# zhuker/lamejs

Measured on NVIDIA H100. Metric: encoded audio seconds/sec (44.1kHz stereo 128kbps CBR), higher is better.
Workload: dtype f64

## Files before the change

lamejs_b200/csrc/k_quant.cuh:

```cuda
#ifndef MP3B200_K_QUANT_CUH
#define MP3B200_K_QUANT_CUH
#include <stddef.h>
#include "mp3_device.cuh"
#include "mp3_tables.h"
#include "k_psy.cuh"

#define Q_LARGE_BITS 100000
#define Q_IXMAX 8206
#define Q_FULL 0xffffffffu

struct GranuleInfoDev {
  int global_gain, part2_3_length, part2_length, big_values, count1, scalefac_compress;
  int table_select[3], region0_count, region1_count, preflag, scalefac_scale, count1table_select, block_type;
  int subblock_gain[4];
  int count1bits, sfbmax, sfbdivide, sfb_lmax, psymax, psy_lmax, sfb_smin, max_nonzero_coeff;
  int scalefac[MP3_SFBMAX];
  int slen[4];
  int part_row;
  int pad_;
  double xrpow_max;
};
struct QuantFrameState {
  int stream, rel_frame;
  int in_old[2], in_step[2];
  int out_old[2], out_step[2];
  int bs_gain0[2], bs_step0[2];
  int used0[2];
  unsigned long long bs_hash[2][2];
  int scfsi[2][4];
  int redo;
  int valid;
};
#define Q_R0(ch) (1 << (ch))
#define Q_R1S(ch) (4 << (ch))
#define Q_R1(ch) (16 << (ch))
#define Q_R0_ANY 3
#define Q_R1_ANY 48
#define Q_R1S_ANY 12
struct GcPrep { float xmin[MP3_SFBMAX]; int have, mnz, block_type; double xrpow_max; };

__device__ unsigned short g_huff_code[1666];
__device__ unsigned char g_huff_len[1666];
__constant__ int c_huff_off[34];
__constant__ int c_huff_xlen[34];
__device__ int g_t32l[16];
__device__ int g_t33l[16];
__constant__ int c_slen1_n[16];
__constant__ int c_slen2_n[16];
__device__ int g_slen_n[2][16];
__device__ int g_scale_tab[2][16];
__device__ unsigned int g_cat_tab[8][256];
__constant__ int c_slen1_tab[16];
__constant__ int c_slen2_tab[16];
__constant__ int c_huf_noesc[15];

static int quant_upload_constants() {
  static const int t32l[16] = {1, 5, 5, 7, 5, 8, 7, 9, 5, 7, 7, 9, 7, 9, 9, 10};
  static const int t33l[16] = {4, 5, 5, 6, 5, 6, 6, 7, 5, 6, 6, 7, 6, 7, 7, 8};
  static const int s1n[16] = {1, 1, 1, 1, 8, 2, 2, 2, 4, 4, 4, 8, 8, 8, 16, 16};
  static const int s2n[16] = {1, 2, 4, 8, 1, 2, 4, 8, 2, 4, 8, 2, 4, 8, 4, 8};
  static const int s1t[16] = {0, 0, 0, 0, 3, 1, 1, 1, 2, 2, 2, 3, 3, 3, 4, 4};
  static const int s2t[16] = {0, 1, 2, 3, 0, 1, 2, 3, 1, 2, 3, 1, 2, 3, 2, 3};
  static const int ss[16] = {0, 18, 36, 54, 54, 36, 54, 72, 54, 72, 90, 72, 90, 108, 108, 126};
  static const int sl[16] = {0, 10, 20, 30, 33, 21, 31, 41, 32, 42, 52, 43, 53, 63, 64, 74};
  static const int hn[15] = {1, 2, 5, 7, 7, 10, 10, 13, 13, 13, 13, 13, 13, 13, 13};
#define UP(sym, src) if (cudaMemcpyToSymbol(sym, src, sizeof(src)) != cudaSuccess) return -100
  UP(g_huff_code, MP3_HUFF_CODE); UP(g_huff_len, MP3_HUFF_LEN); UP(c_huff_off, MP3_HUFF_OFF);
  UP(c_huff_xlen, MP3_HUFF_XLEN);
  UP(g_t32l, t32l); UP(g_t33l, t33l); UP(c_slen1_n, s1n); UP(c_slen2_n, s2n);
  UP(c_slen1_tab, s1t); UP(c_slen2_tab, s2t); UP(c_huf_noesc, hn);
  {
    static int sn[2][16], st[2][16];
    static unsigned int ct[8][256];
    for (int k = 0; k < 16; k++) { sn[0][k] = s1n[k]; sn[1][k] = s2n[k]; st[0][k] = sl[k]; st[1][k] = ss[k]; }
    static const int fam[6] = {1, 2, 5, 7, 10, 13};
    for (int x = 0; x < 16; x++) for (int y = 0; y < 16; y++) {
      const int q = x * 16 + y;
      for (int c = 0; c < 6; c++) {
        const int t1 = fam[c], xl = MP3_HUFF_XLEN[t1];
        unsigned a = 0, b = 0, d = 0;
        if (x < xl && y < xl) {
          const int i = x * xl + y;
          if (c == 0) a = b = d = MP3_HUFF_LEN[MP3_HUFF_OFF[1] + i];
          else if (c == 1) { a = MP3_HUFF_TABLE23[i] >> 16; b = d = MP3_HUFF_TABLE23[i] & 0xffff; }
          else if (c == 2) { a = MP3_HUFF_TABLE56[i] >> 16; b = d = MP3_HUFF_TABLE56[i] & 0xffff; }
          else { a = MP3_HUFF_LEN[MP3_HUFF_OFF[t1] + i]; b = MP3_HUFF_LEN[MP3_HUFF_OFF[t1 + 1] + i]; d = MP3_HUFF_LEN[MP3_HUFF_OFF[t1 + 2] + i]; }
        }
        ct[c][q] = a | (b << 11) | (d << 22);
      }
      { const unsigned a = MP3_HUFF_LARGETBL[q] >> 16, b = MP3_HUFF_LARGETBL[q] & 0xffff; ct[6][q] = a | (b << 11) | (b << 22); }
      ct[7][q] = 0;
    }
    UP(g_slen_n, sn); UP(g_scale_tab, st); UP(g_cat_tab, ct);
  }
#undef UP
  return 0;
}

struct __align__(16) GcWork {
  float xrpow[576];
  short ixw[576];
  short* ixg;
  GranuleInfoDev w, b;
  const Mp3Geo* geo;
  float xmin[MP3_SFBMAX], distort[MP3_SFBMAX];
  int pn_step[MP3_SFBMAX]; float pn_noise[MP3_SFBMAX], pn_noise_log[MP3_SFBMAX];
  int pn_global_gain, pn_sfb_count1;
  unsigned char mode[MP3_SFBMAX + 1];
  short nstart[MP3_SFBMAX], nlen[MP3_SFBMAX];
  int scratch[8];
  double dscratch[4];
  __align__(16) float xr[576];
};
struct __align__(16) WarpShared {
  double ath[6];
  int scfsi[4];
  GcWork wk;
};
#define Q_STRIDE_NOXR ((int)((offsetof(WarpShared, wk) + offsetof(GcWork, xr) + 15) & ~(size_t)15))
static_assert((offsetof(WarpShared, wk) + offsetof(GcWork, xr)) % 16 == 0 && (offsetof(WarpShared, wk) + offsetof(GcWork, xrpow)) % 16 == 0 &&
              (offsetof(WarpShared, wk) + offsetof(GcWork, ixw)) % 16 == 0 && sizeof(WarpShared) % 16 == 0, "rows are moved as 16-byte vectors");
#ifndef Q_SLIM_BLOCKS
#define Q_SLIM_BLOCKS 9
#endif

#define LANE (threadIdx.x & 31)
#ifdef Q_TASKSTAT
__device__ int g_taskstat[1 << 16][8];
#endif
#ifdef Q_STATS
__device__ unsigned long long g_qstats[16];
#define QSTAT(i) do { if (LANE == 0) atomicAdd(&g_qstats[i], 1ull); } while (0)
#else
#define QSTAT(i) do { } while (0)
#endif
#define Q_PRAGMA(x) _Pragma(#x)
#define Q_UNROLL(n) Q_PRAGMA(unroll n)
#ifndef Q_RT_UNROLL
#define Q_RT_UNROLL 1
#endif
#ifndef Q_CB_UNROLL
#define Q_CB_UNROLL 1
#endif
#ifndef Q_CN_UNROLL
#define Q_CN_UNROLL 2
#endif
#ifndef Q_HELPER
#define Q_HELPER __forceinline__
#endif
#ifndef Q_SPEC_START
#define Q_SPEC_START 180
#endif
#ifndef Q_SPEC_STEP
#define Q_SPEC_STEP 32
#endif
#ifndef Q_SPEC_GR1_STEP
#define Q_SPEC_GR1_STEP 2
#endif
#ifndef Q_SPEC_FOLD
#define Q_SPEC_FOLD 1
#endif
#ifndef Q_MIN_BLOCKS
#define Q_MIN_BLOCKS 14
#endif
__device__ __noinline__ double q_log10(double x) { return m3_log10(x); }
__device__ __noinline__ double q_pow(double x, double y) { return m3_pow(x, y); }
__device__ __forceinline__ int wmax(int v) { return __reduce_max_sync(Q_FULL, v); }
__device__ __forceinline__ int wsum(int v) { return __reduce_add_sync(Q_FULL, v); }
__device__ __forceinline__ unsigned wsumu(unsigned v) { return __reduce_add_sync(Q_FULL, v); }

struct RegionClass { int cat; unsigned lin; int t1, t2; };
__device__ Q_HELPER RegionClass region_class(int mx) {
  RegionClass rc;
  rc.lin = 0; rc.t2 = 0;
  if (mx == 0) { rc.cat = 7; rc.t1 = 0; }
  else if (mx <= 15) {
    rc.t1 = c_huf_noesc[mx - 1];
    rc.cat = mx <= 3 ? mx - 1 : (mx <= 5 ? 3 : (mx <= 7 ? 4 : 5));
  } else {
    const int n = 32 - __clz(mx - 15);
    rc.t2 = 24 + (int)((0x7777665432100000ull >> (4 * n)) & 15ull);
    rc.t1 = max(rc.t2 - 8, 16 + (int)((0x7777766554432100ull >> (4 * n)) & 15ull));
    const unsigned la = (unsigned)c_huff_xlen[rc.t1], lb = (unsigned)c_huff_xlen[rc.t2];
    rc.lin = la | (lb << 11) | (lb << 22);
    rc.cat = 6;
  }
  return rc;
}
__device__ __forceinline__ unsigned pair_bits(unsigned w, int cat, unsigned lin) {
  const unsigned x = w & 0xffffu, y = w >> 16;
  const unsigned xe = min(x, 15u), ye = min(y, 15u);
  return __ldg(&g_cat_tab[cat][xe * 16 + ye]) + ((x > 14u) + (y > 14u)) * lin;
}
__device__ Q_HELPER int region_pick(int mx, const RegionClass& rc, int a, int b, int c, int* bits) {
  DOMAIN_MISS(DOM_REGION_MX, mx > Q_IXMAX);
  if (mx > Q_IXMAX) { *bits = Q_LARGE_BITS; return -1; }
  if (mx == 0) return 0;
  int t = rc.t1;
  if (mx <= 15) {
    if (a > b) { a = b; t++; }
    if (a > c) { a = c; t = rc.t1 + 2; }
  } else if (a > b) { a = b; t = rc.t2; }
  *bits += a;
  return t;
}

__device__ __forceinline__ int region_table_w(const short* ix, int begin, int end, int* bits) {
  const int lane = LANE;
  const unsigned* w32 = reinterpret_cast<const unsigned*>(ix);
  const int p0 = (begin >> 1) + lane, p1 = end >> 1;
  unsigned m = 0;
Q_UNROLL(Q_RT_UNROLL)
  for (int p = p0; p < p1; p += 32) m = __vmaxu2(m, w32[p]);
  const int mx = (int)__reduce_max_sync(Q_FULL, max(m & 0xffffu, m >> 16));
  if (mx == 0) return 0;
  const RegionClass rc = region_class(mx);
  unsigned s = 0;
  if (rc.cat == 6) {
Q_UNROLL(Q_RT_UNROLL)
    for (int p = p0; p < p1; p += 32) s += pair_bits(w32[p], 6, rc.lin);
  } else {
    const unsigned int* tab = g_cat_tab[rc.cat];
Q_UNROLL(Q_RT_UNROLL)
    for (int p = p0; p < p1; p += 32) { const unsigned w = w32[p]; s += __ldg(&tab[((w & 0xfu) << 4) | (w >> 16)]); }
  }
#ifdef MP3_DOMAIN_CHECK
  {
    unsigned fa = 0, fb = 0, fc = 0;
    for (int p = p0; p < p1; p += 32) {
      const unsigned v = rc.cat == 6 ? pair_bits(w32[p], 6, rc.lin) : __ldg(&g_cat_tab[rc.cat][((w32[p] & 0xfu) << 4) | (w32[p] >> 16)]);
      fa += v & 0x7ffu; fb += (v >> 11) & 0x7ffu; fc += v >> 22;
    }
    DOMAIN_MISS(DOM_BITSUM_FIELD, fa > 0x7ffu || fb > 0x7ffu || fc > 0x3ffu || wsumu(fa) > 0xffffu || wsumu(fb) > 0xffffu);
  }
#endif
  const unsigned ab = wsumu((s & 0x7ffu) | (((s >> 11) & 0x7ffu) << 16));
  const int c = wsum((int)(s >> 22));
  return region_pick(mx, rc, (int)(ab & 0xffffu), (int)(ab >> 16), c, bits);
}

__device__ __forceinline__ int noquant_count_bits_w(const Mp3Tables* T, const short* ix, GranuleInfoDev* gi, GcWork* wk, bool use_prev, int top) {
  const int lane = LANE;
  const unsigned* w32 = reinterpret_cast<const unsigned*>(ix);
  const int count1 = wmax(top);
  int a1 = 0, a2 = 0, nq = 0;
  const int qmax = count1 >> 2;
  bool stop = false;
#pragma unroll 1
  for (int q0 = 0; q0 < qmax && !stop; q0 += 32) {
    const int q = q0 + lane;
    int bad = 1, v1 = 0, v2 = 0;
    if (q < qmax) {
      const int i = count1 - 4 * q;
      const unsigned wa = w32[(i - 4) >> 1], wb = w32[(i - 2) >> 1];
      if (((wa | wb) & 0xfffefffeu) == 0) {
        bad = 0;
        const int p = (int)(((wa & 1u) << 3) | ((wa >> 16) << 2) | ((wb & 1u) << 1) | (wb >> 16));
        v1 = __ldg(&g_t32l[p]); v2 = __ldg(&g_t33l[p]);
      }
    }
    const unsigned m = __ballot_sync(Q_FULL, bad);
    const int first_bad = m ? __ffs(m) - 1 : 32;
    if (lane >= first_bad) { v1 = 0; v2 = 0; }
    a1 += wsum(v1); a2 += wsum(v2);
    nq += first_bad;
    if (first_bad < 32) stop = true;
  }
  if (nq > qmax) nq = qmax;
  const int bigv = count1 - 4 * nq;
  int bits = a1, c1sel = 0;
  if (a1 > a2) { bits = a2; c1sel = 1; }
  const int count1bits = bits;
  int r0 = gi->region0_count, r1 = gi->region1_count;
  int ts0 = gi->table_select[0], ts1 = gi->table_select[1], ts2 = gi->table_select[2];
  if (bigv != 0) {
    int b1, b2;
    const int bt = gi->block_type;
    if (bt == BT_SHORT) {
      b1 = 3 * T->sfb_s[3];
      b2 = bigv;
    } else if (bt == BT_NORM) {
      b1 = r0 = T->bv_scf[bigv - 2];
      b2 = r1 = T->bv_scf[bigv - 1];
      b2 = T->sfb_l[b1 + b2 + 2];
      b1 = T->sfb_l[b1 + 1];
    } else {
      r0 = 7; r1 = 22 - 1 - 7 - 1;
      b1 = T->sfb_l[7 + 1];
      b2 = bigv;
    }
    b1 = min(b1, bigv);
    b2 = min(b2, bigv);
    if (bt == BT_NORM && b2 < bigv) { QSTAT(15); ts2 = region_table_w(ix, b2, bigv, &bits); }
    if (0 < b1) { QSTAT(15); ts0 = region_table_w(ix, 0, b1, &bits); }
    if (b1 < b2) { QSTAT(15); ts1 = region_table_w(ix, b1, b2, &bits); }
  }
  __syncwarp();
  if (lane == 0) {
    gi->count1 = count1; gi->count1table_select = c1sel; gi->count1bits = count1bits; gi->big_values = bigv;
    gi->region0_count = r0; gi->region1_count = r1;
    gi->table_select[0] = ts0; gi->table_select[1] = ts1; gi->table_select[2] = ts2;
    if (use_prev) {
      int sc = 0;
      if (bigv != 0 && gi->block_type == BT_NORM) {
        if (bigv >= 576) sc = 22;
        else { sc = T->geo[0].sfb_of_line[bigv]; if (T->sfb_l[sc] != bigv) sc++; }
      }
      wk->pn_sfb_count1 = sc;
    }
  }
  __syncwarp();
  return bits;
}

__device__ __forceinline__ int pretab_of(int sfb) { return sfb < 22 ? (int)((0x2fe95400000ull >> (2 * sfb)) & 3ull) : 0; }

__device__ __forceinline__ int sfb_step(const GranuleInfoDev* gi, const GcWork* wk, int sfb) {
  return gi->global_gain - ((gi->scalefac[sfb] + (gi->preflag != 0 ? pretab_of(sfb) : 0)) << (gi->scalefac_scale + 1)) -
         gi->subblock_gain[wk->geo->window[sfb]] * 8;
}

template <bool use_prev>
__device__ __forceinline__ int count_bits_w(const Mp3Tables* T, GcWork* wk, GranuleInfoDev* gi, short* ix) {
  const int lane = LANE;
  const double istep = (double)T->ipow20[gi->global_gain];
  if (gi->xrpow_max > T->ixmax_over_istep[gi->global_gain]) return Q_LARGE_BITS;
  const int sfbmax = gi->block_type == BT_SHORT ? 38 : 21;
  const int mnz = gi->max_nonzero_coeff;
  unsigned* iw32 = reinterpret_cast<unsigned*>(ix);
  const int i0h = min(576, ((mnz + 2) >> 1) << 1) >> 1;
  if (!use_prev) {
    const int qend = (mnz + 1) & ~1;
    int top = 0;
Q_UNROLL(Q_CB_UNROLL)
    for (int p = lane; p < 288; p += 32) {
      unsigned v = 0;
      if (2 * p < qend) {
        const float2 xp = *reinterpret_cast<const float2*>(&wk->xrpow[2 * p]);
        double x0 = (double)xp.x * istep, x1 = (double)xp.y * istep;
        x0 += (double)__ldg(&T->adj43[js_trunc<DOM_TRUNC_QUANT>(x0)]);
        x1 += (double)__ldg(&T->adj43[js_trunc<DOM_TRUNC_QUANT>(x1)]);
        v = (unsigned)js_trunc<DOM_TRUNC_QUANT>(x0) | ((unsigned)js_trunc<DOM_TRUNC_QUANT>(x1) << 16);
        DOMAIN_MISS(DOM_PACK_SEARCH, x0 >= 32768.0 || x1 >= 32768.0);
        if (v != 0 && p < i0h) top = 2 * p + 2;
      }
      iw32[p] = v;
    }
    __syncwarp();
    return noquant_count_bits_w(T, ix, gi, wk, false, top);
  }
  const bool prev_data_use = use_prev && (gi->global_gain == wk->pn_global_gain);
  const bool calc_step = prev_data_use || gi->block_type == BT_NORM;
  int term = sfbmax + 1;
#pragma unroll 1
  for (int s0 = 0; s0 <= sfbmax; s0 += 32) {
    const int sfb = s0 + lane;
    int md = 0, trunc_here = 0;
    if (sfb <= sfbmax) {
      const int jst = wk->geo->start[sfb];
      const int step = calc_step ? sfb_step(gi, wk, sfb) : -1;
      if (prev_data_use && wk->pn_step[sfb] == step) md = 0;
      else {
        if (jst + wk->geo->width[sfb] > mnz) trunc_here = 1;
        md = (use_prev && wk->pn_sfb_count1 > 0 && sfb >= wk->pn_sfb_count1 && wk->pn_step[sfb] > 0 && step >= wk->pn_step[sfb]) ? 2 : 1;
      }
      wk->mode[sfb] = (unsigned char)md;
      wk->nstart[sfb] = jst;
    }
    const unsigned m = __ballot_sync(Q_FULL, trunc_here);
    if (m && term == sfbmax + 1) term = s0 + __ffs(m) - 1;
  }
  __syncwarp();
  int zero_from = 576;
  if (term <= sfbmax) {
    const int term_len = mnz - wk->nstart[term] + 1;
    zero_from = term_len > 0 ? ((term_len & 1) ? mnz : mnz + 1) : mnz;
    if (lane == 0) wk->mode[term] = 1;
  }
  __syncwarp();
  const double compare01 = T->cmp01_over_istep[gi->global_gain];
  int top = 0;
Q_UNROLL(Q_CB_UNROLL)
  for (int p = lane; p < 288; p += 32) {
    const int i = 2 * p;
    unsigned v;
    if (i >= zero_from) { v = 0; iw32[p] = 0; }
    else {
      const int md = wk->mode[wk->geo->sfb_of_line[i]];
      const bool z1 = (i + 1) >= zero_from;
      if (md == 0) {
        v = iw32[p];
        if (z1) { v &= 0xffffu; iw32[p] = v; }
      } else {
        const float2 xp = *reinterpret_cast<const float2*>(&wk->xrpow[i]);
        unsigned v0, v1;
        if (md == 2) { v0 = (compare01 > (double)xp.x) ? 0u : 1u; v1 = (compare01 > (double)xp.y) ? 0u : 1u; }
        else {
          double x0 = (double)xp.x * istep, x1 = (double)xp.y * istep;
          x0 += (double)__ldg(&T->adj43[js_trunc<DOM_TRUNC_QUANT>(x0)]);
          x1 += (double)__ldg(&T->adj43[js_trunc<DOM_TRUNC_QUANT>(x1)]);
          v0 = (unsigned)js_trunc<DOM_TRUNC_QUANT>(x0); v1 = (unsigned)js_trunc<DOM_TRUNC_QUANT>(x1);
          DOMAIN_MISS(DOM_PACK_OUTER, x0 >= 32768.0 || x1 >= 32768.0);
        }
        if (z1) v1 = 0;
        v = v0 | (v1 << 16);
        iw32[p] = v;
      }
    }
    if (v != 0 && p < i0h) top = 2 * p + 2;
  }
  __syncwarp();
  return noquant_count_bits_w(T, ix, gi, wk, use_prev, top);
}

struct NoiseRes { int over_count; double over_SSD, max_noise; int bits; };
__device__ __forceinline__ void calc_noise_w(const Mp3Tables* T, GcWork* wk, const GranuleInfoDev* gi, const short* ix, NoiseRes* res) {
  const int lane = LANE;
  const int psymax = gi->psymax, mnz = gi->max_nonzero_coeff;
  int first_trunc = psymax;
#pragma unroll 1
  for (int s0 = 0; s0 < psymax; s0 += 32) {
    const int sfb = s0 + lane;
    int crosses = 0;
    if (sfb < psymax) {
      const int j = wk->geo->start[sfb], w = wk->geo->width[sfb];
      if (wk->pn_step[sfb] == sfb_step(gi, wk, sfb)) wk->nlen[sfb] = -1;
      else { wk->nstart[sfb] = (short)j; wk->nlen[sfb] = (short)(w >> 1); crosses = (j + w) > mnz; }
    }
    const unsigned m = __ballot_sync(Q_FULL, crosses);
    if (m && first_trunc == psymax) first_trunc = s0 + __ffs(m) - 1;
  }
  __syncwarp();
  if (lane == 0 && first_trunc < psymax) {
    int j = wk->geo->start[first_trunc];
#pragma unroll 1
    for (int sfb = first_trunc; sfb < psymax; sfb++) {
      const int w = wk->geo->width[sfb];
      if (wk->nlen[sfb] < 0) { j += w; continue; }
      int l = w >> 1;
      if ((j + w) > mnz) { const int us = mnz - j + 1; l = us > 0 ? us >> 1 : 0; }
      wk->nstart[sfb] = (short)j; wk->nlen[sfb] = (short)l;
      j += 2 * l;
    }
  }
  __syncwarp();
  int over = 0, ssd = 0; double mxn = -20.0;
#pragma unroll 1
  for (int s0 = 0; s0 < psymax; s0 += 32) {
    const int sfb = s0 + lane;
    if (sfb < psymax) {
      const int s = sfb_step(gi, wk, sfb);
      const bool cached = wk->nlen[sfb] < 0;
      double noise;
      if (cached) noise = (double)wk->pn_noise[sfb];
      else {
        const double step = (double)T->pow20[s + MP3_QMAX2];
        int j = wk->nstart[sfb];
        noise = 0;
Q_UNROLL(Q_CN_UNROLL)
        for (int l = wk->nlen[sfb]; l > 0; l--, j += 2) {
          const float2 x = *reinterpret_cast<const float2*>(&wk->xr[j]);
          const unsigned q0 = reinterpret_cast<const unsigned short*>(ix)[j], q1 = reinterpret_cast<const unsigned short*>(ix)[j + 1];
          double temp;
          temp = fabs((double)x.x) - (double)__ldg(&T->pow43[q0]) * step; noise += temp * temp;
          temp = fabs((double)x.y) - (double)__ldg(&T->pow43[q1]) * step; noise += temp * temp;
        }
        wk->pn_step[sfb] = s;
        { f32s t; t = noise; wk->pn_noise[sfb] = t.v; }
      }
      noise = noise / (double)wk->xmin[sfb];
      { f32s t; t = noise; wk->distort[sfb] = t.v; }
      if (cached) noise = (double)wk->pn_noise_log[sfb];
      else {
        noise = q_log10(js_dmax(noise, 1E-20));
        { f32s t; t = noise; wk->pn_noise_log[sfb] = t.v; }
      }
      if (noise > 0.0) {
        int tmp = js_trunc<DOM_TRUNC_NOISE>(noise * 10 + .5);
        if (tmp < 1) tmp = 1;
        ssd += tmp * tmp;
        over++;
      }
      mxn = js_dmax(mxn, noise);
    }
  }
#pragma unroll 1
  for (int o = 16; o > 0; o >>= 1) {
    const double other = __shfl_xor_sync(Q_FULL, mxn, o);
    mxn = js_dmax(mxn, other);
  }
  over = wsum(over);
  if (lane == 0) wk->pn_global_gain = gi->global_gain;
  __syncwarp();
  res->over_count = over; res->over_SSD = (double)wsum(ssd); res->max_noise = mxn;
}

__device__ __forceinline__ bool scale_bitcount_w(GranuleInfoDev* gi) {
  const int lane = LANE;
  int* scalefac = gi->scalefac;
  const bool is_short = gi->block_type == BT_SHORT;
  const int sfbmax = gi->sfbmax, sfbdivide = gi->sfbdivide;
  __syncwarp();
  if (!is_short && 0 == gi->preflag) {
    const bool in = lane >= 11 && lane < 21;
    const int pt = pretab_of(lane);
    const bool ok = !in || scalefac[lane] >= pt;
    if (__all_sync(Q_FULL, ok)) {
      __syncwarp();
      if (in) scalefac[lane] -= pt;
      if (lane == 0) gi->preflag = 1;
      __syncwarp();
    }
  }
  int m1 = 0, m2 = 0;
#pragma unroll 1
  for (int sfb = lane; sfb < sfbmax; sfb += 32) {
    const int v = scalefac[sfb];
    if (sfb < sfbdivide) m1 = max(m1, v); else m2 = max(m2, v);
  }
  m1 = wmax(m1); m2 = wmax(m2);
  int key = Q_LARGE_BITS * 16 + 15;
  if (lane < 16 && m1 < __ldg(&g_slen_n[0][lane]) && m2 < __ldg(&g_slen_n[1][lane])) key = __ldg(&g_scale_tab[is_short ? 1 : 0][lane]) * 16 + lane;
  key = __reduce_min_sync(Q_FULL, key);
  const int p2 = key >> 4;
  if (lane == 0) { gi->part2_length = p2; if (p2 != Q_LARGE_BITS) gi->scalefac_compress = key & 15; }
  __syncwarp();
  return p2 == Q_LARGE_BITS;
}

__device__ __forceinline__ bool scale_bitcount_lsf_w(GranuleInfoDev* gi) {
  const int lane = LANE;
  const bool is_short = gi->block_type == BT_SHORT;
  __syncwarp();
  int m0 = 0, m1 = 0, m2 = 0, m3 = 0;
  const int n = is_short ? 36 : 21;
#pragma unroll 1
  for (int i = lane; i < n; i += 32) {
    const int v = gi->scalefac[i];
    const int p = is_short ? i / 9 : (i < 6 ? 0 : (i - 6) / 5 + 1);
    if (p == 0) m0 = max(m0, v); else if (p == 1) m1 = max(m1, v); else if (p == 2) m2 = max(m2, v); else m3 = max(m3, v);
  }
  m0 = wmax(m0); m1 = wmax(m1); m2 = wmax(m2); m3 = wmax(m3);
  const bool over = m0 > 15 || m1 > 15 || m2 > 7 || m3 > 7;
  if (!over && lane == 0) {
    const int s1 = m0 ? 32 - __clz(m0) : 0, s2 = m1 ? 32 - __clz(m1) : 0, s3 = m2 ? 32 - __clz(m2) : 0, s4 = m3 ? 32 - __clz(m3) : 0;
    gi->slen[0] = s1; gi->slen[1] = s2; gi->slen[2] = s3; gi->slen[3] = s4;
    gi->part_row = is_short ? 1 : 0;
    gi->scalefac_compress = (((s1 * 5) + s2) << 4) + (s3 << 2) + s4;
    gi->part2_length = is_short ? 9 * (s1 + s2 + s3 + s4) : 6 * s1 + 5 * (s2 + s3 + s4);
  }
  __syncwarp();
  return over;
}
__device__ __forceinline__ bool scale_bitcount_any_w(GranuleInfoDev* gi, int mode_gr) {
  return mode_gr == 2 ? scale_bitcount_w(gi) : scale_bitcount_lsf_w(gi);
}

__device__ __forceinline__ bool loop_break_w(const GranuleInfoDev* gi, const GcWork* wk) {
  bool nz = true;
#pragma unroll 1
  for (int sfb = LANE; sfb < gi->sfbmax; sfb += 32)
    if (gi->scalefac[sfb] + gi->subblock_gain[wk->geo->window[sfb]] == 0) nz = false;
  return __all_sync(Q_FULL, nz);
}

__device__ __forceinline__ void scale_xrpow_w(GcWork* wk, GranuleInfoDev* gi, double f34) {
  const int lane = LANE;
  const int sfbmax = gi->sfbmax;
  float mx = 0.0f;
#pragma unroll 1
  for (int p = lane; p < 288; p += 32) {
    const int sfb = wk->geo->sfb_of_line[2 * p];
    if (sfb < sfbmax && wk->mode[sfb]) {
      float2* xp = reinterpret_cast<float2*>(&wk->xrpow[2 * p]);
      float2 x = *xp;
      f32s v0, v1; v0.v = x.x; v1.v = x.y;
      v0 *= f34; v1 *= f34;
      x.x = v0.v; x.y = v1.v;
      *xp = x;
      mx = fmaxf(mx, fmaxf(v0.v, v1.v));
    }
  }
#pragma unroll 1
  for (int o = 16; o > 0; o >>= 1) mx = fmaxf(mx, __shfl_xor_sync(Q_FULL, mx, o));
  if (lane == 0 && (double)mx > gi->xrpow_max) gi->xrpow_max = (double)mx;
  __syncwarp();
}

__device__ __noinline__ bool balance_escalate_w(const Mp3Tables* T, GcWork* wk) {
  const int lane = LANE;
  GranuleInfoDev* gi = &wk->w;
  int* flag = &wk->scratch[0];
  bool status = true;
  const int scale_now = gi->scalefac_scale, is_short_blk = gi->block_type == BT_SHORT;
  __syncwarp();
  if (T->noise_shaping > 1) {
    if (0 == scale_now) {
      {
        const int sfbmax = gi->sfbmax, pre = gi->preflag;
#pragma unroll 1
        for (int sfb = lane; sfb < sfbmax; sfb += 32) {
          int s = gi->scalefac[sfb];
          if (pre != 0) s += pretab_of(sfb);
          const int odd = (s & 1) != 0;
// ... 1524 lines not shown
```

Baseline: 57860.

## Fuse three region table selections into shared warp passes over big values

Replaces three separate region_table_w calls, each scanning its own span of the big-values area, with two fused warp loops over the whole area. The first loop takes per-region maxima, the second sums pair_bits for all three regions with packed region classes, and warp reductions then feed region_pick. This is meant to cut repeated loop overhead and warp syncs per count_bits call. In exchange, every lane evaluates three masked accumulators per pair, there is extra packing logic, and the table_select writes are now guarded by which regions were actually counted.

```diff
diff --git a/lamejs_b200/csrc/k_quant.cuh b/lamejs_b200/csrc/k_quant.cuh
--- a/lamejs_b200/csrc/k_quant.cuh
+++ b/lamejs_b200/csrc/k_quant.cuh
@@ -187,6 +187,15 @@
   }
   return rc;
 }
+__device__ __forceinline__ unsigned rc_pack(const RegionClass& rc) {
+  return (unsigned)rc.cat | ((unsigned)rc.t1 << 3) | ((unsigned)rc.t2 << 8) | ((rc.lin & 15u) << 13) | (((rc.lin >> 11) & 15u) << 17);
+}
+__device__ __forceinline__ unsigned rc_lin(unsigned k) { return ((k >> 13) & 15u) | ((k >> 17) & 15u) * ((1u << 11) | (1u << 22)); }
+__device__ __forceinline__ RegionClass rc_unpack(unsigned k) {
+  RegionClass rc;
+  rc.cat = (int)(k & 7u); rc.t1 = (int)((k >> 3) & 31u); rc.t2 = (int)((k >> 8) & 31u); rc.lin = rc_lin(k);
+  return rc;
+}
 __device__ __forceinline__ unsigned pair_bits(unsigned w, int cat, unsigned lin) {
   const unsigned x = w & 0xffffu, y = w >> 16;
   const unsigned xe = min(x, 15u), ye = min(y, 15u);
@@ -272,7 +281,7 @@
   if (a1 > a2) { bits = a2; c1sel = 1; }
   const int count1bits = bits;
   int r0 = gi->region0_count, r1 = gi->region1_count;
-  int ts0 = gi->table_select[0], ts1 = gi->table_select[1], ts2 = gi->table_select[2];
+  int ts0 = 0, ts1 = 0, ts2 = 0, counted = 0;
   if (bigv != 0) {
     int b1, b2;
     const int bt = gi->block_type;
@@ -291,15 +300,54 @@
     }
     b1 = min(b1, bigv);
     b2 = min(b2, bigv);
-    if (bt == BT_NORM && b2 < bigv) { QSTAT(15); ts2 = region_table_w(ix, b2, bigv, &bits); }
-    if (0 < b1) { QSTAT(15); ts0 = region_table_w(ix, 0, b1, &bits); }
-    if (b1 < b2) { QSTAT(15); ts1 = region_table_w(ix, b1, b2, &bits); }
+    const int h1 = b1 >> 1, h2 = b2 >> 1, hv = bigv >> 1;
+    unsigned m0 = 0, m1 = 0, m2 = 0;
+Q_UNROLL(Q_RT_UNROLL)
+    for (int p = lane; p < hv; p += 32) {
+      const unsigned w = w32[p];
+      const bool in0 = p < h1, in1 = !in0 && p < h2, in2 = p >= h2;
+      m0 = __vmaxu2(m0, in0 ? w : 0u); m1 = __vmaxu2(m1, in1 ? w : 0u); m2 = __vmaxu2(m2, in2 ? w : 0u);
+    }
+    const int mx0 = (int)__reduce_max_sync(Q_FULL, max(m0 & 0xffffu, m0 >> 16));
+    const int mx1 = (int)__reduce_max_sync(Q_FULL, max(m1 & 0xffffu, m1 >> 16));
+    const int mx2 = (int)__reduce_max_sync(Q_FULL, max(m2 & 0xffffu, m2 >> 16));
+    const unsigned k0 = rc_pack(region_class(mx0)), k1 = rc_pack(region_class(mx1)), k2 = rc_pack(region_class(mx2));
+    unsigned s0 = 0, s1 = 0, s2 = 0;
+Q_UNROLL(Q_RT_UNROLL)
+    for (int p = lane; p < hv; p += 32) {
+      const bool in0 = p < h1, in1 = !in0 && p < h2, in2 = p >= h2;
+      const unsigned k = in0 ? k0 : (in1 ? k1 : k2);
+      const unsigned v = pair_bits(w32[p], (int)(k & 7u), rc_lin(k));
+      s0 += in0 ? v : 0u; s1 += in1 ? v : 0u; s2 += in2 ? v : 0u;
+    }
+#ifdef MP3_DOMAIN_CHECK
+    {
+      unsigned f[3][3] = {};
+      for (int p = lane; p < hv; p += 32) {
+        const int r = p < h1 ? 0 : (p < h2 ? 1 : 2);
+        const unsigned k = r == 0 ? k0 : (r == 1 ? k1 : k2);
+        const unsigned v = pair_bits(w32[p], (int)(k & 7u), rc_lin(k));
+        f[r][0] += v & 0x7ffu; f[r][1] += (v >> 11) & 0x7ffu; f[r][2] += v >> 22;
+      }
+      for (int r = 0; r < 3; r++)
+        DOMAIN_MISS(DOM_BITSUM_FIELD, f[r][0] > 0x7ffu || f[r][1] > 0x7ffu || f[r][2] > 0x3ffu || wsumu(f[r][0]) > 0xffffu || wsumu(f[r][1]) > 0xffffu);
+    }
+#endif
+    const unsigned ab0 = wsumu((s0 & 0x7ffu) | (((s0 >> 11) & 0x7ffu) << 16));
+    const unsigned ab1 = wsumu((s1 & 0x7ffu) | (((s1 >> 11) & 0x7ffu) << 16));
+    const unsigned ab2 = wsumu((s2 & 0x7ffu) | (((s2 >> 11) & 0x7ffu) << 16));
+    const int c0 = wsum((int)(s0 >> 22)), c1 = wsum((int)(s1 >> 22)), c2 = wsum((int)(s2 >> 22));
+    if (b2 < bigv) { QSTAT(15); counted |= 4; ts2 = region_pick(mx2, rc_unpack(k2), (int)(ab2 & 0xffffu), (int)(ab2 >> 16), c2, &bits); }
+    if (0 < b1) { QSTAT(15); counted |= 1; ts0 = region_pick(mx0, rc_unpack(k0), (int)(ab0 & 0xffffu), (int)(ab0 >> 16), c0, &bits); }
+    if (b1 < b2) { QSTAT(15); counted |= 2; ts1 = region_pick(mx1, rc_unpack(k1), (int)(ab1 & 0xffffu), (int)(ab1 >> 16), c1, &bits); }
   }
   __syncwarp();
   if (lane == 0) {
     gi->count1 = count1; gi->count1table_select = c1sel; gi->count1bits = count1bits; gi->big_values = bigv;
     gi->region0_count = r0; gi->region1_count = r1;
-    gi->table_select[0] = ts0; gi->table_select[1] = ts1; gi->table_select[2] = ts2;
+    if (counted & 1) gi->table_select[0] = ts0;
+    if (counted & 2) gi->table_select[1] = ts1;
+    if (counted & 4) gi->table_select[2] = ts2;
     if (use_prev) {
       int sc = 0;
       if (bigv != 0 && gi->block_type == BT_NORM) {
```

After: 57970 (median of 6 runs). Within noise of the previous version (+0.2%).
